# cbacary/MoDeGPT

Measured on AMD Instinct MI355X. Metric: transformer layers compressed/sec (covariance+decomp+rebuild), Llama-3-8B @30%, higher is better.
Workload: dtype f64 from int8 MFMA digit planes, exact route: nine plane pairs + fp64 remainder sums, nothing truncated (error <= 5e-15 per call: fp64 rounding)

## Files before the change

### modegpt_amd/csrc/chol.hip

```cpp
#include "common.hpp"

namespace mdg {

int gemm_f64(int64_t M, int64_t N, int64_t K, double alpha, const void* A, int a_dtype, int64_t sa_i, int64_t sa_k,
             const int64_t* a_rows, const void* B, int b_dtype, int64_t sb_k, int64_t sb_j, double beta, void* C,
             int c_dtype, int64_t ldc, int64_t batch, int64_t a_bs, int64_t b_bs, int64_t c_bs, int flags,
             hipStream_t st);

__device__ __forceinline__ int64_t ceil_div_dev(int64_t a, int64_t b) { return (a + b - 1) / b; }

constexpr int NB = 128;
constexpr int DP = NB + 1;

__device__ __forceinline__ double readlane_f64(double v, int lane) {
  const int lo = __builtin_amdgcn_readlane(__double2loint(v), lane);
  const int hi = __builtin_amdgcn_readlane(__double2hiint(v), lane);
  return __hiloint2double(hi, lo);
}

__device__ __forceinline__ void potrf_diag_block(double* A, int64_t lda, int nb, int64_t k0, double* inv, int* info, double* a, double* xd,
                                                 double* dinv) {
  constexpr int PT = 1024, SB = 16;
  const int tid = threadIdx.x, lane = tid & 63;
  const int wave = __builtin_amdgcn_readfirstlane(tid >> 6);
  const int mi = lane & 15, kq = lane >> 4;
  for (int e = tid; e < NB * NB; e += PT) {
    const int i = e / NB, j = e % NB;
    double v = 0.;
    if (i < nb && j <= i) v = A[(int64_t)i * lda + j];
    else if (i >= nb && i == j) v = 1.;
    a[i * DP + j] = v;
  }
  __syncthreads();

  for (int kb = 0; kb < NB; kb += SB) {
    if (wave == 0) {
      double row[SB], x[SB], rdiag[SB];
      const int li = lane & 15;
#pragma unroll
      for (int c = 0; c < SB; c++) row[c] = (lane < SB && c <= li) ? a[(kb + li) * DP + kb + c] : 0.;
      int first_bad = SB;
#pragma unroll
      for (int j = 0; j < SB; j++) {
        double d = readlane_f64(row[j], j);
        const bool bad = !(d > 0.);
        first_bad = (bad && first_bad == SB) ? j : first_bad;
        d = bad ? 1. : d;
        const double rs = rsqrt(d);
        rdiag[j] = rs;
        row[j] = (li == j) ? d * rs : row[j] * rs;
#pragma unroll
        for (int c = j + 1; c < SB; c++) row[c] -= row[j] * readlane_f64(row[j], c);
      }
      if (first_bad < SB && lane == 0 && kb + first_bad < nb) atomicCAS(info, 0, (int)(k0 + kb + first_bad + 1));
#pragma unroll
      for (int i = 0; i < SB; i++) {
        double sacc = (i == li) ? 1. : 0.;
#pragma unroll
        for (int c = 0; c < i; c++) sacc -= readlane_f64(row[c], i) * x[c];
        x[i] = sacc * rdiag[i];
      }
      if (lane < SB) {
#pragma unroll
        for (int c = 0; c < SB; c++) {
          if (c <= li) a[(kb + li) * DP + kb + c] = row[c];
          dinv[c * (SB + 1) + li] = (c >= li) ? x[c] : 0.;
          if (c > li) a[(kb + li) * DP + kb + c] = x[c];
        }
        xd[kb + li] = x[li];
      }
    }
    __syncthreads();
    const int o = kb + SB, nt = (NB - o) / SB;
    if (wave < nt) {
      const int r0 = o + wave * SB;
      d4 acc = (d4){0., 0., 0., 0.};
#pragma unroll
      for (int k4 = 0; k4 < SB / 4; k4++) {
        const int kk = k4 * 4 + kq;
        acc = __builtin_amdgcn_mfma_f64_16x16x4f64(a[(r0 + mi) * DP + kb + kk], dinv[mi * (SB + 1) + kk], acc, 0, 0, 0);
      }
#pragma unroll
      for (int reg = 0; reg < 4; reg++) a[(r0 + kq + 4 * reg) * DP + kb + mi] = acc[reg];
    }
    __syncthreads();
    const int ntile = nt * (nt + 1) / 2;
    for (int t = wave; t < ntile; t += PT / 64) {
      int ti = 0;
      while ((ti + 1) * (ti + 2) / 2 <= t) ti++;
      const int tj = t - ti * (ti + 1) / 2;
      const int ri = o + ti * SB, rj = o + tj * SB;
      d4 acc;
#pragma unroll
      for (int reg = 0; reg < 4; reg++) acc[reg] = a[(ri + kq + 4 * reg) * DP + rj + mi];
#pragma unroll
      for (int k4 = 0; k4 < SB / 4; k4++) {
        const int kk = k4 * 4 + kq;
        acc = __builtin_amdgcn_mfma_f64_16x16x4f64(-a[(ri + mi) * DP + kb + kk], a[(rj + mi) * DP + kb + kk], acc, 0, 0, 0);
      }
#pragma unroll
      for (int reg = 0; reg < 4; reg++)
        if (ti != tj || mi <= kq + 4 * reg) a[(ri + kq + 4 * reg) * DP + rj + mi] = acc[reg];
    }
    __syncthreads();
  }
  for (int e = tid; e < nb * nb; e += PT) {
    const int i = e / nb, j = e % nb;
    if (j <= i) A[(int64_t)i * lda + j] = a[i * DP + j];
  }
  for (int s2 = SB; s2 < NB; s2 *= 2) {
    const int tps = s2 / SB, ntile = (NB / (2 * s2)) * tps * tps;
    const int pr = wave / (tps * tps), rt = (wave % (tps * tps)) / tps, ct = wave % tps;
    const int C0 = pr * 2 * s2, R0 = C0 + s2;
    d4 acc = (d4){0., 0., 0., 0.};
    if (wave < ntile) {
      const int cj = ct * SB + mi;
      for (int k4 = ct * (SB / 4); k4 < s2 / 4; k4++) {
        const int kk = k4 * 4 + kq;
        const double bv = kk > cj ? a[(C0 + cj) * DP + C0 + kk] : (kk == cj ? xd[C0 + cj] : 0.);
        acc = __builtin_amdgcn_mfma_f64_16x16x4f64(a[(R0 + rt * SB + mi) * DP + C0 + kk], bv, acc, 0, 0, 0);
      }
    }
    __syncthreads();
    if (wave < ntile) {
#pragma unroll
      for (int reg = 0; reg < 4; reg++) a[(R0 + rt * SB + kq + 4 * reg) * DP + C0 + ct * SB + mi] = acc[reg];
    }
    __syncthreads();
    if (wave < ntile) {
      const int ri = rt * SB + mi;
      acc = (d4){0., 0., 0., 0.};
      for (int k4 = 0; k4 < (rt + 1) * (SB / 4); k4++) {
        const int kk = k4 * 4 + kq;
        const double av = ri > kk ? a[(R0 + kk) * DP + R0 + ri] : (ri == kk ? xd[R0 + ri] : 0.);
        acc = __builtin_amdgcn_mfma_f64_16x16x4f64(av, a[(R0 + kk) * DP + C0 + ct * SB + mi], acc, 0, 0, 0);
      }
#pragma unroll
      for (int reg = 0; reg < 4; reg++) a[(C0 + ct * SB + mi) * DP + R0 + rt * SB + kq + 4 * reg] = -acc[reg];
    }
    __syncthreads();
  }
  for (int e = tid; e < NB * NB; e += PT) {
    const int i = e / NB, j = e % NB;
    double v;
    if (i >= nb || j >= nb) v = (i == j) ? 1. : 0.;
    else if (j < i) v = a[j * DP + i];
    else if (j == i) v = xd[i];
    else v = 0.;
    inv[e] = v;
  }
}

__global__ __launch_bounds__(1024) void potrf_diag_kernel(double* A, int64_t lda, int nb, int64_t k0, double* inv, int* info) {
  __shared__ double a[NB * DP];
  __shared__ double xd[NB];
  __shared__ double dinv[16 * 17];
  potrf_diag_block(A, lda, nb, k0, inv, info, a, xd, dinv);
}

template <int MODE>
__global__ __launch_bounds__(1024) void potrf_tile_kernel(double* A, int64_t lda, int64_t r0, int64_t nrows, int64_t k0, int64_t c0,
                                                          int64_t ncols, const double* inv, int next_nb, double* next_inv, int* info) {
  constexpr int PT = 1024, SB = 16;
  __shared__ double a[NB * DP];
  __shared__ double la_xd[MODE == 1 ? NB : 1];
  __shared__ double la_dinv[MODE == 1 ? 16 * 17 : 1];
  const int tid = threadIdx.x, lane = tid & 63;
  const int wave = __builtin_amdgcn_readfirstlane(tid >> 6);
  const int mi = lane & 15, kq = lane >> 4;
  const int64_t ctiles = MODE == 1 ? ceil_div_dev(ncols, NB) : 1;
  const int64_t ti = blockIdx.x / ctiles, tc = blockIdx.x % ctiles;
  const int64_t row0 = r0 + ti * NB, col0 = c0 + tc * NB;
  if (MODE == 1 && row0 + NB - 1 < col0) return;
  const int nr = (int)(r0 + nrows - row0 < NB ? r0 + nrows - row0 : NB);
  const int nc = MODE == 1 ? (int)(c0 + ncols - col0 < NB ? c0 + ncols - col0 : NB) : NB;
  double* Ai = A + row0 * lda + k0;
  const double* Bp = MODE == 1 ? A + col0 * lda + k0 : inv;
  const int64_t ldb = MODE == 1 ? lda : NB;
  for (int e = tid; e < NB * NB; e += PT) {
    const int i = e / NB, j = e % NB;
    a[i * DP + j] = i < nr ? Ai[(int64_t)i * lda + j] : 0.;
  }
  const int ct = wave & 7, rt0 = (wave >> 3) * 4;
  const int bcol = ct * SB + mi;
  __syncthreads();
  d4 acc[4];
#pragma unroll
  for (int t = 0; t < 4; t++) acc[t] = (d4){0., 0., 0., 0.};
  constexpr int KB = 8, NBATCH = NB / 4 / KB;
  double bv[2][KB];
  auto load_b = [&](int kb, double (&v)[KB]) {
#pragma unroll
    for (int u = 0; u < KB; u++) v[u] = bcol < nc ? Bp[(int64_t)bcol * ldb + (kb + u) * 4 + kq] : 0.;
  };
  load_b(0, bv[0]);
#pragma unroll
  for (int q = 0; q < NBATCH; q++) {
    if (MODE == 1 && q + 1 < NBATCH) load_b((q + 1) * KB, bv[(q + 1) & 1]);
    if (MODE == 0 && q > 0) load_b(q * KB, bv[q & 1]);
    if (MODE == 1) __builtin_amdgcn_sched_barrier(0);
#pragma unroll
    for (int u = 0; u < KB; u++) {
      const int kk = (q * KB + u) * 4 + kq;
#pragma unroll
      for (int t = 0; t < 4; t++) acc[t] = __builtin_amdgcn_mfma_f64_16x16x4f64(a[((rt0 + t) * SB + mi) * DP + kk], bv[q & 1][u], acc[t], 0, 0, 0);
    }
  }
  if (MODE == 0) {
    __syncthreads();
#pragma unroll
    for (int t = 0; t < 4; t++)
#pragma unroll
      for (int reg = 0; reg < 4; reg++) {
        const int row = (rt0 + t) * SB + kq + 4 * reg;
        if (row < nr) Ai[(int64_t)row * lda + bcol] = acc[t][reg];
      }
  } else {
    double* C = A + row0 * lda + col0;
    double cold[4][4];
#pragma unroll
    for (int t = 0; t < 4; t++)
#pragma unroll
      for (int reg = 0; reg < 4; reg++) {
        const int row = (rt0 + t) * SB + kq + 4 * reg;
        cold[t][reg] = (row < nr && bcol < nc) ? C[(int64_t)row * lda + bcol] : 0.;
      }
#pragma unroll
    for (int t = 0; t < 4; t++)
#pragma unroll
      for (int reg = 0; reg < 4; reg++) {
        const int row = (rt0 + t) * SB + kq + 4 * reg;
        if (row < nr && bcol < nc) C[(int64_t)row * lda + bcol] = -1.0 * acc[t][reg] + 1.0 * cold[t][reg];
      }
    if (next_nb > 0 && blockIdx.x == 0) {
      __syncthreads();
      potrf_diag_block(A + row0 * lda + col0, lda, next_nb, row0, next_inv, info, a, la_xd, la_dinv);
    }
  }
}

__global__ __launch_bounds__(256) void copy_lower_kernel(const double* src, int64_t lds_, const int64_t* idx, double* dst,
                                                         int64_t ldd, int64_t n, double ridge) {
  const int64_t i = blockIdx.y;
  const int64_t si = idx ? idx[i] : i;
  for (int64_t j = (int64_t)blockIdx.x * 256 + threadIdx.x; j <= i; j += (int64_t)gridDim.x * 256) {
    int64_t sj = idx ? idx[j] : j;
    double v = src[si * lds_ + sj];
    if (j == i) v += ridge;
    dst[i * ldd + j] = v;
  }
}

__global__ __launch_bounds__(256) void place_inv_diag_kernel(const double* inv, double* X, int64_t ldx, int64_t n) {
  const int64_t b = blockIdx.x;
  const double* src = inv + b * NB * NB;
  for (int e = threadIdx.x; e < NB * NB; e += 256) {
    int64_t i = b * NB + e / NB, j = b * NB + e % NB;
    if (i < n && j < n) X[i * ldx + j] = src[e];
  }
}

template <bool SENS>
__global__ __launch_bounds__(256) void lower_colnorm2_kernel(const double* X, int64_t ldx, int64_t n, double* out, const double* u,
                                                             double* sens) {
  __shared__ double red[4][64], red_t[SENS ? 4 : 1][64];
  const int lane = threadIdx.x & 63, wave = threadIdx.x >> 6;
  const int64_t j = (int64_t)blockIdx.x * 64 + lane;
  const int64_t i0 = (int64_t)blockIdx.x * 64;
  double s = 0., t = 0.;
  if (j < n)
    for (int64_t i = i0 + wave; i < n; i += 4)
      if (i >= j) {
        double v = X[i * ldx + j];
        s += v * v;
        if (SENS) t += fabs(v) * u[i];
      }
  red[wave][lane] = s;
  if (SENS) red_t[wave][lane] = t;
  __syncthreads();
  if (wave == 0 && j < n) {
    out[j] = red[0][lane] + red[1][lane] + red[2][lane] + red[3][lane];
    if (SENS) {
      const double tt = red_t[0][lane] + red_t[1][lane] + red_t[2][lane] + red_t[3][lane];
      sens[j] = tt * tt;
    }
  }
}

__global__ __launch_bounds__(256) void sqrt_diag_kernel(const double* C, int64_t ldc, int64_t n, double* d) {
  const int64_t a = (int64_t)blockIdx.x * 256 + threadIdx.x;
  if (a < n) {
    const double c = C[a * ldc + a];
    d[a] = c > 0. ? sqrt(c) : 0.;
  }
}
__global__ __launch_bounds__(256) void lower_abs_rowsum_kernel(const double* X, int64_t ldx, int64_t n, const double* d, double* u) {
  const int lane = threadIdx.x & 63;
  const int64_t b = (int64_t)blockIdx.x * 4 + (threadIdx.x >> 6);
  if (b >= n) return;
  double acc = 0.;
  for (int64_t a = lane; a <= b; a += 64) acc += fabs(X[b * ldx + a]) * d[a];
#pragma unroll
  for (int o = 32; o > 0; o >>= 1) acc += __shfl_xor(acc, o);
  if (lane == 0) u[b] = acc;
}


#ifndef MDG_CHOL_TILE_KERNELS
#define MDG_CHOL_TILE_KERNELS 1
#endif
#ifndef MDG_CHOL_LOOKAHEAD
#define MDG_CHOL_LOOKAHEAD 1
#endif
#ifndef MDG_CHOL_NBO
#define MDG_CHOL_NBO 2048
#endif
constexpr int NBO = MDG_CHOL_NBO;

int potrf_lower(double* A, int64_t n, int64_t lda, double* inv_diag, hipStream_t st) {
  const int64_t nblk = ceil_div(n, NB);
  int* dflag = (int*)(inv_diag + nblk * NB * NB);
  MDG_HIP(hipMemsetAsync(dflag, 0, sizeof(int), st));
  for (int64_t J0 = 0; J0 < n; J0 += NBO) {
    const int64_t Jend = J0 + NBO < n ? J0 + NBO : n;
    bool diag_done = false;
    for (int64_t k0 = J0; k0 < Jend; k0 += NB) {
      const int nb = (int)(n - k0 < NB ? n - k0 : NB);
      double* inv = inv_diag + (k0 / NB) * NB * NB;
      if (!diag_done) hipLaunchKernelGGL(potrf_diag_kernel, dim3(1), dim3(1024), 0, st, A + k0 * lda + k0, lda, nb, k0, inv, dflag);
      diag_done = false;
      MDG_LAUNCH_CHECK();
      const int64_t rest = n - k0 - nb;
      if (rest <= 0) break;
      double* A21 = A + (k0 + nb) * lda + k0;
      const int64_t w = Jend - (k0 + nb);
#if MDG_CHOL_TILE_KERNELS
      hipLaunchKernelGGL(potrf_tile_kernel<0>, dim3((unsigned)ceil_div(rest, NB)), dim3(1024), 0, st, A, lda, k0 + nb, rest, k0,
                         (int64_t)0, (int64_t)0, inv, 0, (double*)nullptr, (int*)nullptr);
      if (w > 0) {
        const int next_nb = (int)(n - (k0 + nb) < NB ? n - (k0 + nb) : NB);
        hipLaunchKernelGGL(potrf_tile_kernel<1>, dim3((unsigned)(ceil_div(rest, NB) * ceil_div(w, NB))), dim3(1024), 0, st, A, lda,
                           k0 + nb, rest, k0, k0 + nb, w, inv, MDG_CHOL_LOOKAHEAD ? next_nb : 0, inv + NB * NB, dflag);
        diag_done = MDG_CHOL_LOOKAHEAD != 0;
      }
      MDG_LAUNCH_CHECK();
#else
      MDG_TRY(gemm_f64(rest, nb, nb, 1.0, A21, MDG_F64, lda, 1, nullptr, inv, MDG_F64, 1, NB, 0.0, A21, MDG_F64, lda, 1,
                       0, 0, 0, 0, st));
      if (w > 0)
        MDG_TRY(gemm_f64(rest, w, nb, -1.0, A21, MDG_F64, lda, 1, nullptr, A21, MDG_F64, 1, lda, 1.0,
                         A + (k0 + nb) * lda + (k0 + nb), MDG_F64, lda, 1, 0, 0, 0, 0, st));
#endif
    }
    const int64_t rest = n - Jend;
    if (rest > 0) {
      const double* Lp = A + Jend * lda + J0;
      MDG_TRY(gemm_f64(rest, rest, Jend - J0, -1.0, Lp, MDG_F64, lda, 1, nullptr, Lp, MDG_F64, 1, lda, 1.0,
                       A + Jend * lda + Jend, MDG_F64, lda, 1, 0, 0, 0, MDG_GEMM_LOWER_ONLY, st));
    }
  }
  return finish_flag(dflag, st, STATUS_NOT_PD, "Cholesky");
}

int tri_inverse_doubling(const double* L, int64_t n, int64_t ldl, const double* inv_diag, double* X, int64_t ldx, double* T,
                         int64_t s_limit, hipStream_t st) {
  const int64_t nblk = ceil_div(n, NB);
  hipLaunchKernelGGL(place_inv_diag_kernel, dim3((unsigned)nblk), dim3(256), 0, st, inv_diag, X, ldx, n);
  MDG_LAUNCH_CHECK();
  for (int64_t s = NB; s < n && s < s_limit; s *= 2) {
    const int64_t full = n / (2 * s);
    const int64_t r0_last = full * 2 * s + s;
    const int64_t pair_stride_L = 2 * s * ldl + 2 * s, pair_stride_X = 2 * s * ldx + 2 * s;
    for (int pass = 0; pass < 2; pass++) {
      int64_t p0, cnt, m;
      if (pass == 0) { p0 = 0; cnt = full; m = s; }
      else { p0 = full; cnt = r0_last < n ? 1 : 0; m = n - r0_last; }
      if (cnt <= 0) continue;
      const int64_t c0 = p0 * 2 * s, r0 = c0 + s;
      MDG_TRY(gemm_f64(m, s, s, 1.0, L + r0 * ldl + c0, MDG_F64, ldl, 1, nullptr, X + c0 * ldx + c0, MDG_F64, ldx, 1,
                       0.0, T, MDG_F64, s, cnt, pair_stride_L, pair_stride_X, s * s, MDG_GEMM_B_LOWER_TRI, st));
      MDG_TRY(gemm_f64(m, s, m, -1.0, X + r0 * ldx + r0, MDG_F64, ldx, 1, nullptr, T, MDG_F64, s, 1, 0.0,
                       X + r0 * ldx + c0, MDG_F64, ldx, cnt, pair_stride_X, s * s, pair_stride_X,
                       MDG_GEMM_A_LOWER_TRI, st));
    }
  }
  return MDG_OK;
}

int chol_inverse_diag(const double* L, int64_t n, int64_t ldl, const double* inv_diag, double* out, double* X,
                      double* T, hipStream_t st, const double* C = nullptr, int64_t ldc = 0, double* sens = nullptr) {
  const int64_t ldx = n;
  MDG_TRY(tri_inverse_doubling(L, n, ldl, inv_diag, X, ldx, T, n, st));
  if (sens) {
    double* d = T;
    double* u = T + n;
    hipLaunchKernelGGL(sqrt_diag_kernel, dim3((unsigned)ceil_div(n, 256)), dim3(256), 0, st, C, ldc, n, d);
    hipLaunchKernelGGL(lower_abs_rowsum_kernel, dim3((unsigned)ceil_div(n, 4)), dim3(256), 0, st, X, ldx, n, d, u);
    hipLaunchKernelGGL(lower_colnorm2_kernel<true>, dim3((unsigned)ceil_div(n, 64)), dim3(256), 0, st, X, ldx, n, out, u, sens);
  } else {
    hipLaunchKernelGGL(lower_colnorm2_kernel<false>, dim3((unsigned)ceil_div(n, 64)), dim3(256), 0, st, X, ldx, n, out,
                       (const double*)nullptr, (double*)nullptr);
  }
  MDG_LAUNCH_CHECK();
  return MDG_OK;
}

#ifndef MDG_CHOL_NBS
#define MDG_CHOL_NBS 2048
#endif
constexpr int NBS = MDG_CHOL_NBS;

size_t potrs_ws_elems(int64_t n, int64_t nrhs) {
  return (size_t)n * NBS + (size_t)n + ((size_t)n * NBS / 4 + NB * NB) + (size_t)n * nrhs;
}

int potrs_lower(const double* L, int64_t n, int64_t ldl, const double* inv_diag, double* X, int64_t nrhs, int64_t ldx,
                double* ws, hipStream_t st) {
  double* Linv = ws;
  double* T = Linv + (size_t)n * NBS + n;
  double* W = T + ((size_t)n * NBS / 4 + NB * NB);
  MDG_TRY(tri_inverse_doubling(L, n, ldl, inv_diag, Linv, NBS, T, NBS, st));
  for (int64_t J0 = 0; J0 < n; J0 += NBS) {
    const int64_t Jend = J0 + NBS < n ? J0 + NBS : n, nbj = Jend - J0;
    MDG_TRY(gemm_f64(nbj, nrhs, nbj, 1.0, Linv + J0 * NBS + J0, MDG_F64, NBS, 1, nullptr, X + J0 * ldx, MDG_F64, ldx, 1, 0.0,
                     W + J0 * nrhs, MDG_F64, nrhs, 1, 0, 0, 0, MDG_GEMM_A_LOWER_TRI, st));
    if (n - Jend > 0)
      MDG_TRY(gemm_f64(n - Jend, nrhs, nbj, -1.0, L + Jend * ldl + J0, MDG_F64, ldl, 1, nullptr, W + J0 * nrhs, MDG_F64, nrhs,
                       1, 1.0, X + Jend * ldx, MDG_F64, ldx, 1, 0, 0, 0, 0, st));
  }
  const int64_t last_J0 = ((n - 1) / NBS) * NBS;
  for (int64_t J0 = last_J0; J0 >= 0; J0 -= NBS) {
    const int64_t Jend = J0 + NBS < n ? J0 + NBS : n, nbj = Jend - J0;
    MDG_TRY(gemm_f64(nbj, nrhs, nbj, 1.0, Linv + J0 * NBS + J0, MDG_F64, 1, NBS, nullptr, W + J0 * nrhs, MDG_F64, nrhs, 1, 0.0,
                     X + J0 * ldx, MDG_F64, ldx, 1, 0, 0, 0, MDG_GEMM_A_UPPER_TRI, st));
    if (J0 > 0)
      MDG_TRY(gemm_f64(J0, nrhs, nbj, -1.0, L + J0 * ldl, MDG_F64, 1, ldl, nullptr, X + J0 * ldx, MDG_F64, ldx, 1, 1.0, W,
                       MDG_F64, nrhs, 1, 0, 0, 0, 0, st));
  }
  return MDG_OK;
}

int copy_lower(const double* src, int64_t ld_src, const int64_t* idx, double* dst, int64_t ldd, int64_t n,
               double ridge, hipStream_t st) {
  MDG_CHECK_ARG(n < 65536 * 4, "copy_lower: n too large");
  unsigned gx = (unsigned)(ceil_div(n, 256) < 64 ? ceil_div(n, 256) : 64);
  hipLaunchKernelGGL(copy_lower_kernel, dim3(gx, (unsigned)n), dim3(256), 0, st, src, ld_src, idx, dst, ldd, n, ridge);
  MDG_LAUNCH_CHECK();
  return MDG_OK;
}

}

using namespace mdg;

extern "C" size_t mdg_potrf_inv_diag_elems(int64_t n) { return (size_t)ceil_div(n, NB) * NB * NB + 16; }

extern "C" int mdg_potrf_lower(double* A, int64_t n, int64_t lda, double* inv_diag, void* stream) {
  MDG_CLEAR();
  MDG_CHECK_ARG(A && inv_diag && n > 0 && lda >= n, "mdg_potrf_lower: bad arguments");
  return potrf_lower(A, n, lda, inv_diag, (hipStream_t)stream);
}

extern "C" size_t mdg_potrs_lower_ws_bytes(int64_t n, int64_t nrhs) {
  if (n <= 0 || nrhs <= 0) return 0;
  return potrs_ws_elems(n, nrhs) * sizeof(double);
}

extern "C" int mdg_potrs_lower(const double* L, int64_t n, int64_t ldl, const double* inv_diag, double* X,
                               int64_t nrhs, int64_t ldx, void* ws, size_t ws_bytes, void* stream) {
  MDG_CLEAR();
  MDG_CHECK_ARG(L && inv_diag && X && n > 0 && nrhs > 0 && ldl >= n && ldx >= nrhs, "mdg_potrs_lower: bad arguments");
  MDG_CHECK_ARG(ws && ws_bytes >= mdg_potrs_lower_ws_bytes(n, nrhs), "mdg_potrs_lower: workspace %zu < required %zu", ws_bytes,
                mdg_potrs_lower_ws_bytes(n, nrhs));
  return potrs_lower(L, n, ldl, inv_diag, X, nrhs, ldx, (double*)ws, (hipStream_t)stream);
}

extern "C" size_t mdg_chol_inverse_diag_ws_bytes(int64_t n) {
  return ((size_t)n * n + (size_t)n * n / 4 + NB * NB) * sizeof(double);
}

extern "C" int mdg_chol_inverse_diag(const double* L, int64_t n, int64_t ldl, const double* inv_diag, double* out,
                                     void* ws, size_t ws_bytes, void* stream) {
  MDG_CLEAR();
  MDG_CHECK_ARG(L && inv_diag && out && n > 0 && ldl >= n, "mdg_chol_inverse_diag: bad arguments");
  MDG_CHECK_ARG(ws && ws_bytes >= mdg_chol_inverse_diag_ws_bytes(n), "mdg_chol_inverse_diag: workspace too small");
  double* X = (double*)ws;
  double* T = X + (size_t)n * n;
  return chol_inverse_diag(L, n, ldl, inv_diag, out, X, T, (hipStream_t)stream);
}

extern "C" size_t mdg_ridge_scores_ws_bytes(int64_t n) {
  return (size_t)n * n * sizeof(double) + mdg_potrf_inv_diag_elems(n) * sizeof(double) +
         mdg_chol_inverse_diag_ws_bytes(n);
}

extern "C" int mdg_ridge_scores(const double* C, int64_t n, int64_t ldc, double ridge, double* scores, double* sens, void* ws,
                                size_t ws_bytes, void* stream) {
  MDG_CLEAR();
  MDG_CHECK_ARG(C && scores && n > 0 && ldc >= n, "mdg_ridge_scores: bad arguments");
  MDG_CHECK_ARG(ws && ws_bytes >= mdg_ridge_scores_ws_bytes(n), "mdg_ridge_scores: workspace %zu < required %zu",
                ws_bytes, mdg_ridge_scores_ws_bytes(n));
  hipStream_t st = (hipStream_t)stream;
  double* Lb = (double*)ws;
  double* inv = Lb + (size_t)n * n;
  double* rest = inv + mdg_potrf_inv_diag_elems(n);
  MDG_TRY(copy_lower(C, ldc, nullptr, Lb, n, n, ridge, st));
  MDG_TRY(potrf_lower(Lb, n, n, inv, st));
  return chol_inverse_diag(Lb, n, n, inv, scores, rest, rest + (size_t)n * n, st, C, ldc, sens);
}
```

Measured before the change: 1.149.

## Overlap diagonal sub-block factorization with trailing updates in potrf diag kernel

Moves the 16x16 diagonal sub-block Cholesky and inverse into a helper run by wave 0 right after it does its trailing-update tile, so the next panel factorization happens in the same phase as the other waves' updates. This removes one barrier per step. The helper also drops lane predication and adds scheduling barriers to limit register pressure. Stores of L back to global memory and of the final inverse are folded into the triangular-inverse doubling loop, and the last level writes inv directly from registers, which removes separate passes and syncs. The cost is a more intricate, order-sensitive schedule: wave 0 carries extra serial work and correctness depends on it updating the next diagonal tile first.

```diff
diff --git a/modegpt_amd/csrc/chol.hip b/modegpt_amd/csrc/chol.hip
--- a/modegpt_amd/csrc/chol.hip
+++ b/modegpt_amd/csrc/chol.hip
@@ -16,6 +16,61 @@
   const int lo = __builtin_amdgcn_readlane(__double2loint(v), lane);
   const int hi = __builtin_amdgcn_readlane(__double2hiint(v), lane);
   return __hiloint2double(hi, lo);
+}
+
+__device__ __forceinline__ int opaque(int v) {
+  asm volatile("" : "+v"(v));
+  return v;
+}
+
+__device__ __forceinline__ void potrf_sub_block(double* a, double* xd, double* dinv, int kb, int nb, int64_t k0, int* info, int lane) {
+  constexpr int SB = 16;
+  double row[SB], x[SB], rdiag[SB];
+  {
+    const double* src = a + (kb + (lane & 15)) * DP + kb;
+#pragma unroll
+    for (int c = 0; c < SB; c++) row[c] = src[c];
+  }
+  int first_bad = SB;
+#pragma unroll
+  for (int j = 0; j < SB; j++) {
+    const int li = opaque(lane & 15);
+    double d = readlane_f64(row[j], j);
+    const bool bad = !(d > 0.);
+    first_bad = (bad && first_bad == SB) ? j : first_bad;
+    d = bad ? 1. : d;
+    const double rs = rsqrt(d);
+    rdiag[j] = rs;
+    row[j] = (li == j) ? d * rs : row[j] * rs;
+#pragma unroll
+    for (int c = j + 1; c < SB; c++) row[c] -= row[j] * readlane_f64(row[j], c);
+    __builtin_amdgcn_sched_barrier(0);
+  }
+  if (first_bad < SB && lane == 0 && kb + first_bad < nb) atomicCAS(info, 0, (int)(k0 + kb + first_bad + 1));
+#pragma unroll
+  for (int c = 0; c < SB; c++) asm volatile("" : "+v"(row[c]));
+#pragma unroll
+  for (int i = 0; i < SB; i++) {
+    const int li = opaque(lane & 15);
+    double sacc = (i == li) ? 1. : 0.;
+#pragma unroll
+    for (int c = 0; c < i; c++) sacc -= readlane_f64(row[c], i) * x[c];
+    x[i] = sacc * rdiag[i];
+    __builtin_amdgcn_sched_barrier(0);
+  }
+  {
+    const int l16 = lane & 15;
+    double* dst = a + (kb + l16) * DP + kb;
+    double xdg = 0.;
+#pragma unroll
+    for (int c = 0; c < SB; c++) {
+      const int li = opaque(l16);
+      dst[c] = (c <= li) ? row[c] : x[c];
+      dinv[c * (SB + 1) + l16] = (c >= li) ? x[c] : 0.;
+      xdg = (c == li) ? x[c] : xdg;
+    }
+    xd[kb + l16] = xdg;
+  }
 }
 
 __device__ __forceinline__ void potrf_diag_block(double* A, int64_t lda, int nb, int64_t k0, double* inv, int* info, double* a, double* xd,
@@ -32,45 +87,10 @@
     a[i * DP + j] = v;
   }
   __syncthreads();
-
-  for (int kb = 0; kb < NB; kb += SB) {
-    if (wave == 0) {
-      double row[SB], x[SB], rdiag[SB];
-      const int li = lane & 15;
-#pragma unroll
-      for (int c = 0; c < SB; c++) row[c] = (lane < SB && c <= li) ? a[(kb + li) * DP + kb + c] : 0.;
-      int first_bad = SB;
-#pragma unroll
-      for (int j = 0; j < SB; j++) {
-        double d = readlane_f64(row[j], j);
-        const bool bad = !(d > 0.);
-        first_bad = (bad && first_bad == SB) ? j : first_bad;
-        d = bad ? 1. : d;
-        const double rs = rsqrt(d);
-        rdiag[j] = rs;
-        row[j] = (li == j) ? d * rs : row[j] * rs;
-#pragma unroll
-        for (int c = j + 1; c < SB; c++) row[c] -= row[j] * readlane_f64(row[j], c);
-      }
-      if (first_bad < SB && lane == 0 && kb + first_bad < nb) atomicCAS(info, 0, (int)(k0 + kb + first_bad + 1));
-#pragma unroll
-      for (int i = 0; i < SB; i++) {
-        double sacc = (i == li) ? 1. : 0.;
-#pragma unroll
-        for (int c = 0; c < i; c++) sacc -= readlane_f64(row[c], i) * x[c];
-        x[i] = sacc * rdiag[i];
-      }
-      if (lane < SB) {
-#pragma unroll
-        for (int c = 0; c < SB; c++) {
-          if (c <= li) a[(kb + li) * DP + kb + c] = row[c];
-          dinv[c * (SB + 1) + li] = (c >= li) ? x[c] : 0.;
-          if (c > li) a[(kb + li) * DP + kb + c] = x[c];
-        }
-        xd[kb + li] = x[li];
-      }
-    }
-    __syncthreads();
+  if (wave == 0) potrf_sub_block(a, xd, dinv, 0, nb, k0, info, lane);
+  __syncthreads();
+
+  for (int kb = 0; kb + SB < NB; kb += SB) {
     const int o = kb + SB, nt = (NB - o) / SB;
     if (wave < nt) {
       const int r0 = o + wave * SB;
@@ -85,7 +105,7 @@
     }
     __syncthreads();
     const int ntile = nt * (nt + 1) / 2;
-    for (int t = wave; t < ntile; t += PT / 64) {
+    for (int t = wave == 0 ? 0 : wave; t < (wave == 0 ? 1 : ntile); t += PT / 64 - 1) {
       int ti = 0;
       while ((ti + 1) * (ti + 2) / 2 <= t) ti++;
       const int tj = t - ti * (ti + 1) / 2;
@@ -102,16 +122,26 @@
       for (int reg = 0; reg < 4; reg++)
         if (ti != tj || mi <= kq + 4 * reg) a[(ri + kq + 4 * reg) * DP + rj + mi] = acc[reg];
     }
+    if (wave == 0) potrf_sub_block(a, xd, dinv, o, nb, k0, info, lane);
     __syncthreads();
   }
-  for (int e = tid; e < nb * nb; e += PT) {
-    const int i = e / nb, j = e % nb;
-    if (j <= i) A[(int64_t)i * lda + j] = a[i * DP + j];
-  }
   for (int s2 = SB; s2 < NB; s2 *= 2) {
+    const bool first = s2 == SB, last = s2 * 2 == NB;
     const int tps = s2 / SB, ntile = (NB / (2 * s2)) * tps * tps;
     const int pr = wave / (tps * tps), rt = (wave % (tps * tps)) / tps, ct = wave % tps;
     const int C0 = pr * 2 * s2, R0 = C0 + s2;
+    if (last) {
+      for (int e = tid; e < NB * NB; e += PT) {
+        const int i = e / NB, j = e % NB;
+        if (i >= s2 && j < s2) continue;
+        double v;
+        if (i >= nb || j >= nb) v = (i == j) ? 1. : 0.;
+        else if (j < i) v = a[j * DP + i];
+        else if (j == i) v = xd[i];
+        else v = 0.;
+        inv[e] = v;
+      }
+    }
     d4 acc = (d4){0., 0., 0., 0.};
     if (wave < ntile) {
       const int cj = ct * SB + mi;
@@ -119,6 +149,12 @@
         const int kk = k4 * 4 + kq;
         const double bv = kk > cj ? a[(C0 + cj) * DP + C0 + kk] : (kk == cj ? xd[C0 + cj] : 0.);
         acc = __builtin_amdgcn_mfma_f64_16x16x4f64(a[(R0 + rt * SB + mi) * DP + C0 + kk], bv, acc, 0, 0, 0);
+      }
+    }
+    if (first) {
+      for (int e = tid; e < NB * NB; e += PT) {
+        const int i = e / NB, j = e % NB;
+        if (i < nb && j <= i) A[(int64_t)i * lda + j] = a[i * DP + j];
       }
     }
     __syncthreads();
@@ -135,19 +171,18 @@
         const double av = ri > kk ? a[(R0 + kk) * DP + R0 + ri] : (ri == kk ? xd[R0 + ri] : 0.);
         acc = __builtin_amdgcn_mfma_f64_16x16x4f64(av, a[(R0 + kk) * DP + C0 + ct * SB + mi], acc, 0, 0, 0);
       }
-#pragma unroll
-      for (int reg = 0; reg < 4; reg++) a[(C0 + ct * SB + mi) * DP + R0 + rt * SB + kq + 4 * reg] = -acc[reg];
-    }
-    __syncthreads();
-  }
-  for (int e = tid; e < NB * NB; e += PT) {
-    const int i = e / NB, j = e % NB;
-    double v;
-    if (i >= nb || j >= nb) v = (i == j) ? 1. : 0.;
-    else if (j < i) v = a[j * DP + i];
-    else if (j == i) v = xd[i];
-    else v = 0.;
-    inv[e] = v;
+      if (!last) {
+#pragma unroll
+        for (int reg = 0; reg < 4; reg++) a[(C0 + ct * SB + mi) * DP + R0 + rt * SB + kq + 4 * reg] = -acc[reg];
+      } else {
+#pragma unroll
+        for (int reg = 0; reg < 4; reg++) {
+          const int i = R0 + rt * SB + kq + 4 * reg, j = C0 + ct * SB + mi;
+          inv[i * NB + j] = i < nb ? -acc[reg] : 0.;
+        }
+      }
+    }
+    if (!last) __syncthreads();
   }
 }
 
```

New measurement: 1.147. No clear change (-0.2%).
